# learner-shx/SVG-IR

Measured on AMD Instinct MI355X. Metric: Gaussian-surfels/sec fwd+bwd @800x800 (1 view), higher is better.
Workload: dtype f32; 1 GPU; cfg2: rgss path, P=200000 surfels, 800x800, SH degree 3, S=5, VS=0, fwd+bwd, one view per step per GPU (BASELINE.json configs[1] = cfg2 at N=1; configs[3] = cfg4, view r on rank r, at N>1); num_rendered=673008, parallelism=view-parallel x1, per_rank_cpus=not pinned

## Files before the change

### svg-ir_amd/csrc/render_fwd.hip

```cpp
#include <algorithm>

#include "common.hpp"
#include "shade_tables.hpp"
#include "stage.hpp"
#include "pairstage.hpp"
#include "dev_trace.hpp"

namespace svgir {

namespace {

#ifndef CULL_THREADS
#define CULL_THREADS 256
#endif
constexpr int CT = CULL_THREADS, CNW = CT / 64;

__global__ void __launch_bounds__(CT) cull_kernel(const RenderArgs a) {
    __shared__ uint32_t wcnt[CNW][4];
    const uint32_t tile_u = xcd_tile_of_work(blockIdx.x, a.gx, a.gy);
    if (tile_u == ORDER_NONE) return;
    const int tile = (int)tile_u;
    const uint32_t r0 = a.ranges[2 * tile], r1 = a.ranges[2 * tile + 1];
    const int len = (int)(r1 - r0);
    const int t = threadIdx.x, lane = t & 63, wave = t >> 6;
    const int tx = tile % a.gx, ty = tile / a.gx;
    if (!a.bg_in_render && t < 256 && (a.zero_a || a.zero_b)) {
        const int px = tx * TILE + (t & 15), py = ty * TILE + (t >> 4);
        if (px < a.W && py < a.H) write_zero_planes(a, (size_t)a.W * py + px, (size_t)a.W * a.H);
    }
    if (len == 0) {
        if (t < 4) { a.sub_total[4 * tile + t] = 0u; a.sub_count[4 * tile + t] = 0u; a.sub_ndump[4 * tile + t] = 0u; }
        const int px = tx * TILE + (t & 15), py = ty * TILE + (t >> 4);
        if (!a.bg_in_render && t < 256 && px < a.W && py < a.H) write_background(a, (size_t)a.W * py + px, (size_t)a.W * a.H);
        return;
    }
    const float X0 = (float)(tx * TILE), Y0 = (float)(ty * TILE);
    const float4* __restrict__ rec4 = reinterpret_cast<const float4*>(a.rec);
    uint2* __restrict__ out = a.sub_list + (size_t)4 * r0;
    const unsigned long long lt_mask = (lane == 0) ? 0ull : (~0ull >> (64 - lane));
    uint32_t run[4] = {0u, 0u, 0u, 0u};
    uint32_t gid_n = t < len ? a.point_list[r0 + t] : 0u;
    uint32_t gid_nn = CT + t < len ? a.point_list[r0 + CT + t] : 0u;
    float4 A_n = rec4[(size_t)gid_n * 6], B_n = rec4[(size_t)gid_n * 6 + 1];
    for (int base = 0; base < len; base += CT) {
        const int i = base + t;
        bool m[4] = {false, false, false, false};
        const uint32_t gid = gid_n;
        const float4 A = A_n, B = B_n;
        gid_n = gid_nn;
        if (base + CT < len) { A_n = rec4[(size_t)gid_n * 6]; B_n = rec4[(size_t)gid_n * 6 + 1]; }
        gid_nn = base + 2 * CT + t < len ? a.point_list[r0 + base + 2 * CT + t] : 0u;
        if (i < len) {
            const SplatCull sc = cull_prepare(A.x, A.y, A.z, A.w, B.x, B.y);
#pragma unroll
            for (int w = 0; w < 4; w++) {
                const float x0 = X0 + (float)((w & 1) * 8), y0 = Y0 + (float)((w >> 1) * 8);
                m[w] = cull_test(sc, x0, y0, x0 + 7.f, y0 + 7.f);
            }
        }
        unsigned long long mask[4];
#pragma unroll
        for (int w = 0; w < 4; w++) {
            mask[w] = __ballot(m[w]);
            if (lane == 0) wcnt[wave][w] = (uint32_t)__popcll(mask[w]);
        }
        __syncthreads();
        const uint2 e = make_uint2(gid, (uint32_t)i);
#pragma unroll
        for (int w = 0; w < 4; w++) {
            uint32_t before = 0, all = 0;
#pragma unroll
            for (int v = 0; v < CNW; v++) { const uint32_t c = wcnt[v][w]; all += c; before += v < wave ? c : 0u; }
            if (m[w]) out[(size_t)w * len + run[w] + before + (uint32_t)__popcll(mask[w] & lt_mask)] = e;
            run[w] += all;
        }
        __syncthreads();
    }
    if (t < 4) {
        const uint32_t mine = t == 0 ? run[0] : t == 1 ? run[1] : t == 2 ? run[2] : run[3];
        a.sub_total[4 * tile + t] = mine;
        if (mine == 0u) { a.sub_count[4 * tile + t] = 0u; a.sub_ndump[4 * tile + t] = 0u; }
        if (a.queue_order) dispatch_publish_tile(a, tile, blockIdx.x & 7u, run, t);
    }
}

__global__ void __launch_bounds__(64) dispatch_publish_kernel(const RenderArgs a) {
    uint32_t n_ne;
    (void)dispatch_item(a, 0u, (int)threadIdx.x, &n_ne);
}

template <int S, int VC, bool SVGSS, int WPE>
__global__ void __launch_bounds__(64) __attribute__((amdgpu_waves_per_eu(WPE < 2 ? WPE : 2, WPE)))
render_fwd_kernel(const RenderArgs a) {
    using PG = PairGeom<S, VC>;
    constexpr int CH = PG::CH, PF = PG::PF;
    constexpr int KB = StageGeom<S, VC>::KB, NP = KB / 2;
    static_assert(KB == 4 && CH % KB == 0, "a group = the 4 K-rows of one MFMA");
    extern __shared__ __attribute__((aligned(16))) char smem[];
    float* sD = reinterpret_cast<float*>(smem);
    uint2* sQ = reinterpret_cast<uint2*>(smem + PG::off_q);
    float* sW = reinterpret_cast<float*>(smem + PG::off_w);
    float* sP = reinterpret_cast<float*>(smem + PG::off_p);
    constexpr int PS = PG::PS;

    uint32_t n_ne;
    const uint32_t sid = dispatch_item(a, blockIdx.x, (int)threadIdx.x, &n_ne);
    if (sid == ORDER_NONE) {
        if (a.queue_order) dispatch_idle(a, blockIdx.x - n_ne, gridDim.x - n_ne, (int)threadIdx.x);
        return;
    }
    const int tile = (int)(sid >> 2), sub = (int)(sid & 3u);
    const int tx = tile % a.gx, ty = tile / a.gx;
    const int lane = threadIdx.x;
    const int bx = tx * TILE + (sub & 1) * 8, by = ty * TILE + (sub >> 1) * 8;
    const int px = bx + (lane & 7), py = by + (lane >> 3);
    const bool inside = px < a.W && py < a.H;
    const float pxf = (float)px, pyf = (float)py;
    const f32x2 pxx = {pxf, pxf}, pyy = {pyf, pyf};
    const uint32_t r0 = a.ranges[2 * tile], r1 = a.ranges[2 * tile + 1];
    const int len = (int)(r1 - r0);
    if (len == 0) {
        if (a.bg_in_render && !a.dump_only && inside) {
            write_background(a, (size_t)a.W * py + px, (size_t)a.W * a.H);
// ... 47 lines not shown
#pragma unroll
            for (int mt = 0; mt < 4; mt++) {
                float* d = sP + nq * PS + 16 * mt + 4 * kq;
                d[0] = vacc[mt].x; d[1] = vacc[mt].y; d[2] = vacc[mt].z; d[3] = vacc[mt].w;
            }
            wave_lds_sync();
#pragma unroll
            for (int c = 0; c < VC; c++) vfv[c] = sP[c * PS + lane];
        }
        wave_lds_sync();
    };
    auto chan = [&](int c) -> float { return chv[c]; };
    auto vchan = [&](int c) -> float { return vfv[c]; };
    uint32_t last_walk = 0;

    constexpr int NST = 8 + S + VC;
    const uint32_t dump_base = a.sub_slot_base[sid];
    uint32_t ndump = 0;
    auto dump_state = [&](uint32_t j, bool last) {
        const bool slot = dump_base + j < a.slot_cap;
        if (!slot && !last) return;
        gather_acc();
        if (!slot) return;
        float* d = a.seg_state + ((size_t)(dump_base + j) * NST) * 64 + lane;
        d[0] = T; d[64] = chan(0); d[128] = chan(1); d[192] = chan(2);
        d[256] = surface ? chan(3) : 0.f; d[320] = surface ? chan(4) : 0.f; d[384] = surface ? chan(5) : 0.f; d[448] = D;
#pragma unroll
        for (int ch = 0; ch < S; ch++) d[(8 + ch) * 64] = chan(6 + ch);
#pragma unroll
        for (int ch = 0; ch < VC; ch++) d[(8 + S + ch) * 64] = vchan(ch);
    };

    uint32_t head = 0;
    if (total > 0) {
        for (int i = lane; i < (CH / 2) * PF / 4; i += 64) reinterpret_cast<float4*>(sD)[i] = make_float4(0.f, 0.f, 0.f, 0.f);
        auto load_entries = [&](int b) -> uint2 {
            const int i = b * CH + lane;
            return (lane < CH && i < total) ? list[i] : make_uint2(0u, 0u);
        };
        const int nb = (total + CH - 1) / CH;
        if (lane < CH) sQ[lane] = load_entries(0);
        uint2 e_next = load_entries(1);
        wave_lds_sync();
        PairMap<S, VC> pmap;
        pmap.init(lane);
        PairRegs<S, VC> sr;
        pair_stage_load<S, VC, CH>(sr, pmap, min(CH, total), [&](int s) { return sQ[s].x; }, lane, a.rec, a.features, a.vfeatures);
        bool wave_done = __all(done);
        int nflush = 0;
        auto flush_weights = [&](int bprev) {
            if (lane < nflush) {
                const float* wp = sW + (bprev & 1) * (4 * CH) + lane;
                const float wsum = (wp[0] + wp[CH]) + (wp[2 * CH] + wp[3 * CH]);
                if (wsum != 0.f && !a.dump_only) atomic_add_f32(&a.out_weights[sQ[(bprev & 1) * CH + lane].x], wsum);
            }
        };
        int b = 0;
        for (; b < nb && !wave_done; b++) {
            const int m = min(CH, total - b * CH);
            const uint2* q_cur = sQ + (b & 1) * CH;
            float* w_cur = sW + (b & 1) * (4 * CH);
            wave_lds_sync();
            pair_stage_store<S, VC, CH>(sr, pmap, sD, m, lane);
            flush_weights(b - 1);
            wave_lds_sync();
            if (lane < CH) sQ[((b + 1) & 1) * CH + lane] = e_next;
            e_next = load_entries(b + 2);
            wave_lds_sync();
            if (b + 1 < nb) {
                const uint2* q_nxt = sQ + ((b + 1) & 1) * CH;
                pair_stage_load<S, VC, CH>(sr, pmap, min(CH, total - (b + 1) * CH), [&](int s) { return q_nxt[s].x; }, lane, a.rec,
                                       a.features, a.vfeatures);
            }
            DEV_TRACE_MARK(1);
            int nproc = m;
            for (int c0 = 0; c0 < m; c0 += KB) {
                f32x2 dx[NP], dy[NP];
                f32x4 Gd[NP], Ge[NP];
                float pw[KB], al[KB];
#pragma unroll
                for (int p = 0; p < NP; p++) {
                    const f32x4* P = reinterpret_cast<const f32x4*>(sD + ((c0 >> 1) + p) * PF);
                    const f32x4 G0 = P[0], G1 = P[1], G2 = P[2];
                    Gd[p] = P[3]; Ge[p] = P[4];
                    dx[p] = G0.xy - pxx; dy[p] = G0.zw - pyy;
                    const f32x2 pw2 = pair_power2(G1.xy, G2.xy, G1.zw, dx[p], dy[p]);
                    f32x2 a2;
                    {
#pragma clang fp contract(off)
                        a2 = G2.zw * exp_nonpos2(pw2);
                    }
                    pw[2 * p] = pw2.x; pw[2 * p + 1] = pw2.y;
                    al[2 * p] = fminf(0.99f, a2.x); al[2 * p + 1] = fminf(0.99f, a2.y);
                }
                bool pre[KB];
#pragma unroll
                for (int k = 0; k < KB; k++) pre[k] = pw[k] <= 0.0f && al[k] >= (1.0f / 255.0f);
                float w[KB];
#pragma unroll
                for (int k = 0; k < KB; k++) {
                    const bool live = pre[k] && !done;
                    const float test_T = T * (1.f - al[k]);
                    const bool stop = test_T < 0.0001f;
                    const bool pass = live && !stop;
                    done = done || (live && stop);
                    w[k] = pass ? al[k] * T : 0.f;
// ... 49 lines not shown
                    }
                    wave_lds_sync();
                    {
                        const float bch = sD[((c0 >> 1) + (kq >> 1)) * PF + PG::CH_OFF + (kq & 1) * PG::CHP + nq];
    #pragma unroll
                        for (int mt = 0; mt < 4; mt++)
                            acc[mt] = __builtin_amdgcn_mfma_f32_16x16x4f32(sP[kq * PS + 16 * mt + nq], bch, acc[mt], 0, 0, 0);
                    }
                    if (VC > 0) {
    #pragma unroll
                        for (int k = 0; k < KB; k++) {
                            const float bv = sD[((c0 + k) >> 1) * PF + PG::V_OFF + (k & 1) * PG::VB + kq * PG::VCP + nq];
    #pragma unroll
                            for (int mt = 0; mt < 4; mt++)
                                vacc[mt] = __builtin_amdgcn_mfma_f32_16x16x4f32(sP[(4 + k * 4 + kq) * PS + 16 * mt + nq], bv, vacc[mt], 0, 0, 0);
                        }
                    }
                    wave_lds_sync();
                }
                {
                    const bool o1 = (lane & 1) != 0, o2 = (lane & 2) != 0;
                    const float t01 = (o1 ? w[1] : w[0]) + dpp_f32<0xB1>(o1 ? w[0] : w[1]);
                    const float t23 = (o1 ? w[3] : w[2]) + dpp_f32<0xB1>(o1 ? w[2] : w[3]);
                    float u = (o2 ? t23 : t01) + dpp_f32<0x4E>(o2 ? t01 : t23);
                    u += dpp_f32<0x114>(u);
                    u += dpp_f32<0x118>(u);
                    if ((lane & 12) == 12) w_cur[(lane >> 4) * CH + c0 + (lane & 3)] = u;
                }
                if (__all(done)) { wave_done = true; nproc = min(m, c0 + KB); break; }
            }
            nflush = nproc;
            head += (uint32_t)m;
            DEV_TRACE_MARK(2);
            if (!wave_done && (head & (uint32_t)(SEG - 1)) == 0u) dump_state(ndump++, false);
        }
        wave_lds_sync();
        flush_weights(b - 1);
    }
    if (lane == 0 && !a.dump_only) {
        a.sub_count[sid] = head; a.sub_ndump[sid] = ndump;
        const uint32_t nseg = head != 0 ? min((head + (uint32_t)SEG - 1u) / (uint32_t)SEG, ndump + 1u) : 0u;
        if (nseg != 0) {
            uint32_t* cnt = a.seg_block + (tile >> 8) * SEG_BLOCK_STRIDE;
            const int lc = seg_class(head - (nseg - 1u) * (uint32_t)SEG);
            if (nseg > 1u || lc == 0) atomicAdd(cnt, nseg - (lc == 0 ? 0u : 1u));
            if (lc != 0) atomicAdd(cnt + lc, 1u);
        }
    }
    if (head != 0 && ndump != 0) dump_state(ndump, true);
    else gather_acc();

    if (inside && !a.dump_only) {
        const size_t N_ = (size_t)a.W * a.H;
        const size_t pid = (size_t)a.W * py + px;
        if (a.bg_in_render) write_zero_planes(a, pid, N_);
        T = fminf((float)(1 - 0.000001), T);
        a.final_T[pid] = T;
        a.n_contrib[pid] = last_walk ? (int32_t)(list[last_walk - 1u].y + 1u) : 0;
        a.out_color[pid] = chan(0) + T * a.bg[0];
        a.out_color[N_ + pid] = chan(1) + T * a.bg[1];
        a.out_color[2 * N_ + pid] = chan(2) + T * a.bg[2];
#pragma unroll
        for (int ch = 0; ch < S; ch++) a.out_feature[ch * N_ + pid] = chan(6 + ch);
#pragma unroll
        for (int ch = 0; ch < VC; ch++) a.out_vfeature[ch * N_ + pid] = vchan(ch);
        a.out_normal[pid] = surface ? chan(3) : 0.f;
        a.out_normal[N_ + pid] = surface ? chan(4) : 0.f;
        a.out_normal[2 * N_ + pid] = surface ? chan(5) : 0.f;
        a.out_depth[pid] = normalize_depth ? D / (1.f - T) : D + T * 10.f;
        a.out_opacity[pid] = 1.f - T;
        a.final_D[pid] = D;
    }
    DEV_TRACE_MARK(3);
    DEV_TRACE_END(0, (unsigned)total, head, blockIdx.x);
}

__global__ void __launch_bounds__(64) contrib_prepass_kernel(const RenderArgs a) {
    __shared__ __attribute__((aligned(16))) float sQ[2][32][12];
    __shared__ uint32_t sG[2][64];
    uint32_t n_ne;
    const uint32_t sid = dispatch_item(a, blockIdx.x, (int)threadIdx.x, &n_ne);
    if (sid == ORDER_NONE) return;
    const int tile = (int)(sid >> 2), sub = (int)(sid & 3u);
    const uint32_t r0 = a.ranges[2 * tile], r1 = a.ranges[2 * tile + 1];
    const int len = (int)(r1 - r0);
    if (len == 0) return;
    const int total = (int)a.sub_total[sid];
    if (total == 0) return;
    const int lane = threadIdx.x;
    const int tx = tile % a.gx, ty = tile / a.gx;
    const int px = tx * TILE + (sub & 1) * 8 + (lane & 7), py = ty * TILE + (sub >> 1) * 8 + (lane >> 3);
    const float pxf = (float)px, pyf = (float)py;
    const f32x2 pxx = {pxf, pxf}, pyy = {pyf, pyf};
    const uint2* __restrict__ list = a.sub_list + (size_t)4 * r0 + (size_t)sub * len;
// ... 219 lines not shown
```

### svg-ir_amd/csrc/api.hip

```cpp
#include <algorithm>
#include <cstdarg>
#include <cstdio>
#include <atomic>
#include <cstdlib>
#include <ctime>
#include <memory>
#include <mutex>
#include <string>
#include <vector>

#include "common.hpp"
#include "geom_bwd.hpp"
#include "workload_history.hpp"
#include "depth_sort_plan.hpp"

using namespace svgir;

namespace {

thread_local std::string g_err;
std::atomic<bool> g_prof{false};
WorkloadHistory g_history;
unsigned long long* pinned_words(size_t n) {
    void* ptr = nullptr;
// ... 308 lines not shown
                        sp.training ? 52 : 64, sp.training, p->S, p->VS);
        if (!sp.viewmatrix) return fail(SVGIR_ERR_INVALID, "fused shading needs sp.viewmatrix (packed view-space normals)");
    }
    return 0;
}

CapKey workload_key(const svgir_params* p) {
    int dev_id = 0;
    (void)hipGetDevice(&dev_id);
    return CapKey{dev_id, p->W, p->H, p->P, p->S, p->variant == SVGIR_SVGSS ? p->VS : 0, p->variant, p->workload_scope};
}

bool bin_capacity(size_t bytes, const char* image_blob, int W, int H, int nstate, Wait how, const hipStream_t* stream, ViewCounts* vc) {
    const bool compact = bin_bytes_compact(bytes);
    if (compact || how != Wait::kCaps)
        *vc = resolve_view(image_blob, image_layout(const_cast<char*>(image_blob), W, H).counters, how, stream, compact);
    if (compact) return vc->known && vc->cap_slots >= 0;
    vc->cap_R = binning_capacity_from_bytes(bytes, view_grid(W, H).T, nstate);
    vc->cap_slots = -1;
    return true;
}

template <class A> void camera_args(A& a, const svgir_params* p) {
    a.P = p->P; a.D = p->D; a.M = p->M; a.means3D = p->means3D; a.shs = p->colors_precomp ? nullptr : p->shs;
    a.scales = p->scales; a.rotations = p->rotations; a.view = p->viewmatrix; a.proj = p->projmatrix; a.campos = p->cam_pos;
    a.scale_modifier = p->scale_modifier; a.tanx = p->tan_fovx; a.tany = p->tan_fovy; a.cfg = cfg_ref(p);
    a.focal_x = p->W / (2.0f * p->tan_fovx); a.focal_y = p->H / (2.0f * p->tan_fovy);
}

RenderArgs render_args(const svgir_params* p, const ViewGrid& v, const GeomLayout& G, const ImageLayout& I, const BinLayout& B, int fin) {
    const bool svgss = p->variant == SVGIR_SVGSS;
    RenderArgs ra{};
    ra.W = v.W; ra.H = v.H; ra.gx = v.gx; ra.gy = v.gy; ra.S = p->S; ra.VS = svgss ? p->VS : 0;
    ra.ranges = I.ranges; ra.point_list = B.val[fin]; ra.rec = G.rec; ra.features = p->features; ra.vfeatures = p->vfeatures;
    ra.bg = p->background; ra.cfg = cfg_ref(p);
    ra.sub_list = B.sub_list; ra.sub_total = I.sub_total; ra.sub_order = I.sub_order; ra.sub_count = I.sub_count; ra.sub_ndump = I.sub_ndump;
    ra.sub_pair_base = I.sub_pair_base; ra.sub_slot_base = I.sub_slot_base; ra.disp_ctr = I.disp_ctr; ra.disp_item = I.disp_item;
    ra.seg_list = B.seg_list; ra.seg_desc = B.seg_desc; ra.seg_count = I.counters; ra.seg_block = I.seg_block; ra.seg_state = B.seg_state;
    ra.slot_cap = (uint32_t)std::min<size_t>(B.slot_cap, 0xffffffffu);
    ra.order_n = (int)order_entries(v.gx, v.gy);
    ra.bg_in_render = render_specialised(p->S, ra.VS, svgss) ? 1 : 0;
    ra.final_T = I.final_T; ra.final_D = I.final_D; ra.n_contrib = I.n_contrib;
    return ra;
}
}

extern "C" {

int svgir_abi_version(void) { return SVGIR_ABI_VERSION; }
size_t svgir_geom_bytes(int32_t P) { return geom_layout(nullptr, P).bytes; }
size_t svgir_image_bytes(int32_t W, int32_t H) { return image_layout(nullptr, W, H).bytes; }
size_t svgir_binning_bytes(int32_t R, int32_t W, int32_t H, int32_t S, int32_t VS) {
    return bin_layout(nullptr, binning_capacity(R), view_grid(W, H).T, seg_nstate(S, VS)).bytes;
}
size_t svgir_image_ncontrib_offset(int32_t W, int32_t H) { return image_layout(nullptr, W, H).ncontrib_off; }
size_t svgir_image_ranges_offset(int32_t W, int32_t H) {
    const ImageLayout I = image_layout((char*)256, W, H);
    return (size_t)((char*)I.ranges - (char*)256);
}
size_t svgir_binning_point_list_offset(size_t binning_bytes, const char* image_blob, int32_t W, int32_t H, int32_t S, int32_t VS) {
    const int T = view_grid(W, H).T, nstate = seg_nstate(S, VS);
    ViewCounts vc;
    if (!bin_capacity(binning_bytes, image_blob, W, H, nstate, Wait::kCaps, nullptr, &vc)) return (size_t)-1;
    const BinLayout B = bin_layout((char*)256, vc.cap_R, T, nstate);
    return (size_t)((char*)B.val[tile_sort_plan(T).passes & 1] - (char*)256);
}
// ... 595 lines not shown
```

### svg-ir_amd/csrc/common.hpp

```cpp
#pragma once
#include <hip/hip_runtime.h>
#include <stddef.h>
#include <stdint.h>
#include <stdlib.h>

#include <algorithm>

#include "../../include/svgir_raster.h"
#include "wave.hpp"

namespace svgir {

constexpr int TILE = 16;
constexpr int BLOCK = 256;
constexpr int REC = 24;

enum RecField {
    R_X = 0, R_Y = 1, R_CX = 2, R_CY = 3,
    R_CZ = 4, R_OP = 5, R_DEPTH = 6, R_DA = 7,
    R_J0 = 8, R_J1 = 9, R_J2 = 10, R_J3 = 11,
    R_DB = 12, R_R = 13, R_G = 14, R_B = 15,
    R_NX = 16, R_NY = 17, R_NZ = 18, R_IU = 19,
    R_IV = 20, R_IBASE = 21, R_RECT = 22, R_PAD2 = 23
};
// ... 47 lines not shown
    g.key[0] = (uint32_t*)take(p * 4);
    g.key[1] = (uint32_t*)take(p * 4);
    g.idx[0] = (uint32_t*)take(p * 4);
    g.idx[1] = (uint32_t*)take(p * 4);
    g.offsets = (uint32_t*)take(p * 4);
    g.radix_tbl = (uint32_t*)take(radix_table_words(P) * 4);
    g.radix_wtbl = (uint32_t*)take((size_t)256 * sort_blocks(P) * 4);
    g.counters = (uint32_t*)take(16);
    g.key_top = (uint32_t*)take((p + 63) / 64 * 4);
    g.needed = (uint8_t*)take(p);
    g.shade_list = (uint32_t*)take(p * 4);
    g.shade_work = (uint32_t*)take(((size_t)scan_blocks(P) + 2) * 4);
    g.bytes = off;
    return g;
}

constexpr uint32_t ORDER_NONE = 0xffffffffu;
#if defined(__HIPCC__)
__host__ __device__
#endif
inline uint32_t xcd_of_tile(int tx, int ty) { return (uint32_t)((tx >> 2) + 3 * (ty >> 2)) & 7u; }
inline size_t order_entries(int gx, int gy) {
    size_t cnt[8] = {0, 0, 0, 0, 0, 0, 0, 0};
    for (int by = 0; 4 * by < gy; by++)
        for (int bx = 0; 4 * bx < gx; bx++) cnt[xcd_of_tile(4 * bx, 4 * by)] += (size_t)std::min(4, gx - 4 * bx) * (size_t)std::min(4, gy - 4 * by);
    size_t m = 0;
    for (size_t c : cnt) m = std::max(m, c);
    return std::max((size_t)8 * 4 * m, (size_t)4 * gx * gy);
}

#if defined(__HIPCC__)
__host__ __device__
#endif
inline uint32_t xcd_tile_of_work(uint32_t q, int gx, int gy) {
    const int c = (int)(q & 7u), nbx = (gx + 3) >> 2, nby = (gy + 3) >> 2;
    const int wl = gx - 4 * (nbx - 1);
    uint32_t rem = q >> 3;
    for (int by = 0; by < nby; by++) {
        const int bh = gy - 4 * by < 4 ? gy - 4 * by : 4;
        const int r = (c - 3 * by) & 7;
        const int nblk = nbx > r ? (nbx - r + 7) / 8 : 0;
        const bool has_last = nblk > 0 && ((nbx - 1 - r) & 7) == 0;
        const uint32_t cnt = (uint32_t)(bh * (4 * nblk - (has_last ? 4 - wl : 0)));
        if (rem >= cnt) { rem -= cnt; continue; }
        const int k = (int)(rem / (uint32_t)(bh * 4));
        const int bx = r + 8 * k;
        const uint32_t within = rem - (uint32_t)(k * bh * 4);
        const int bw = bx == nbx - 1 ? wl : 4;
        return (uint32_t)((4 * by + (int)(within / (uint32_t)bw)) * gx + 4 * bx + (int)(within % (uint32_t)bw));
    }
    return ORDER_NONE;
}

constexpr int SEG_CLASSES = 5, SEG_BLOCK_STRIDE = 8;

struct ImageLayout {
    float* final_T;
    float* final_D;
    int32_t* n_contrib;
    uint32_t* ranges;
    uint32_t* seg_block;
    uint32_t* sub_total;
    uint32_t* sub_order;
    uint32_t* sub_count;
    uint32_t* sub_ndump;
    uint32_t* sub_pair_base;
    uint32_t* sub_slot_base;
    uint32_t* counters;
    uint32_t* disp_ctr;
    uint32_t* disp_item;
    size_t ncontrib_off;
    size_t bytes;
};
constexpr int DISP_NCLS = 64, DISP_SHARDS = 8, DISP_STEP = 16;
constexpr int DISP_CTR_WORDS = DISP_NCLS * DISP_SHARDS + 2;
inline ImageLayout image_layout(char* base, int W, int H) {
    ImageLayout im;
    size_t off = 0;
    auto take = [&](size_t bytes) { char* p = base ? base + off : nullptr; off += align_up(bytes); return p; };
    const size_t N = (size_t)W * H;
    const size_t T = (size_t)((W + TILE - 1) / TILE) * ((H + TILE - 1) / TILE);
    im.final_T = (float*)take(N * 4);
    im.final_D = (float*)take(N * 4);
    im.ncontrib_off = off;
// ... 133 lines not shown
    return i < c.len && c.ptr[i] > 0.f;
}
#endif

struct ShadeTables {
    const float* env = nullptr; float4* env_tab = nullptr; int ntexel = 0, softplus = 0;
    int Ns = 0; float4* lat_tab = nullptr;
    float* zero = nullptr; int nzero = 0;
#if defined(__HIPCC__)
    __host__ __device__
#endif
    int entries() const { return env ? (ntexel > (lat_tab ? Ns : 0) ? ntexel : (lat_tab ? Ns : 0)) : 0; }
};

struct PreArgs {
    int P, D, M, W, H, gx, gy;
    const float *means3D, *shs, *colors_precomp, *opacities, *scales, *rotations, *cov3D_precomp;
    const float *view, *proj, *campos, *patchbbox;
    float scale_modifier, tanx, tany, focal_x, focal_y;
    CfgRef cfg;
    float* rec; float* cov3D; uint32_t* clamped; uint32_t* tiles; uint32_t* key; uint32_t* idx; int32_t* radii;
    float* out_weights;
    uint8_t* needed;
    uint32_t* span;
    ShadeTables tabs; int pblocks;
    uint32_t* zero_words; int n_zero_words;
    int spec_top; uint32_t* key_top;
    uint32_t* prefilter_violation;
    const float* features; int embed_S;
};

struct RenderArgs {
    int W, H, gx, gy, S, VS;
    const uint32_t* ranges; const uint32_t* point_list;
    const float* rec; const float* features; const float* vfeatures;
    const float* bg;
    CfgRef cfg;
    uint2* sub_list; uint32_t* sub_total; uint32_t* sub_order; uint32_t* sub_count;
    uint32_t* sub_ndump; uint32_t* seg_list; SegDesc* seg_desc; uint32_t* seg_count; uint32_t* seg_block; float* seg_state;
    uint32_t* sub_pair_base; uint32_t* sub_slot_base; uint32_t slot_cap;
    int bg_in_render;
    int order_n;
    int hi_fill;
    int dump_only;
    float *final_T, *final_D; int32_t* n_contrib;
    float *out_color, *out_normal, *out_depth, *out_opacity, *out_feature, *out_vfeature, *out_weights;
    float *zero_a, *zero_b;
    uint8_t* needed;
    int queue_order; uint32_t* disp_ctr; uint32_t* disp_item;
    int publish; uint32_t pub_tag, pub_cap_R, pub_magic; long long pub_cap_slots; unsigned long long* pub_host;
};

struct RenderBwdArgs {
    int W, H, gx, gy, S, VS;
    const uint32_t* ranges; const uint32_t* point_list;
    const float* rec; const float* features; const float* vfeatures;
    const float* bg;
    CfgRef cfg; int backward_geometry;
    const uint2* sub_list; const uint32_t* sub_count;
    const uint32_t* sub_ndump; const uint32_t* seg_list; const SegDesc* seg_desc; const uint32_t* seg_count; const float* seg_state; int seg_cap;
    const float *final_T, *final_D; const int32_t* n_contrib;
    const float *g_color, *g_normal, *g_depth, *g_opacity, *g_feature, *g_vfeature;
    float *dL_dmean2D, *dL_dconic, *dL_dopacity, *dL_dcolor, *dL_dfeature, *dL_dvfeature, *dL_dnormal, *dL_ddepth;
    float* grad_rows; uint32_t* row_of; uint32_t rows_cap;
    uint4* clear; size_t clear_n16;
};
// ... 205 lines not shown
```

### svg-ir_amd/csrc/stage.hpp

```cpp
#pragma once
#include "common.hpp"

namespace svgir {

template <int S, int VC>
struct StageGeom {
    static constexpr int S4 = (S + 3) / 4 * 4;
    static constexpr int NFD = REC + S4 + VC * 4;
    static constexpr int NF4 = (NFD / 4) | 1;
    static constexpr int NF = NF4 * 4;
    static constexpr int C4 = 6 + VC;
    static constexpr int CH = NF <= 48 ? 64 : 32;
    static constexpr int QN = 2 * CH;
#ifndef FWD_KB_V
#define FWD_KB_V 4
#endif
#ifndef FWD_KB_P
#define FWD_KB_P 4
#endif
    static constexpr int KB = VC > 0 ? FWD_KB_V : FWD_KB_P;
#ifndef FWD_WPE_V
#define FWD_WPE_V 2
#endif
#ifndef FWD_WPE_P
// ... 6 lines not shown
    static_assert(SEG % CH == 0, "segment boundaries must fall on staging-batch boundaries");
    static_assert(CH % KB == 0, "a staging batch is a whole number of blend batches");
};

#if defined(__HIPCC__)
__device__ __forceinline__ float pair_power(float a, float b, float c, float dx, float dy) {
    float s, m;
    {
#pragma clang fp contract(off)
        s = a * dx * dx + c * dy * dy;
        m = b * dx * dy;
    }
    return __builtin_fmaf(-0.5f, s, -m);
}

__device__ __forceinline__ float exp_nonpos(float x) {
    const float L2E_HI = 1.44269502162933349609375f;
    const float L2E_LO = 1.92596299112661746e-8f;
    const float t = x * L2E_HI;
    float r = __builtin_fmaf(x, L2E_HI, -t);
    r = __builtin_fmaf(x, L2E_LO, r);
    const float e = __builtin_amdgcn_exp2f(t);
    return __builtin_fmaf(e, r * 0.693147182464599609375f, e);
}

struct SplatCull {
    float mx, my, a, b, c, tau2, ia, ic;
    bool degenerate;
};
__device__ __forceinline__ SplatCull cull_prepare(float mx, float my, float a, float b, float c, float op) {
    SplatCull s;
    s.mx = mx; s.my = my; s.a = a; s.b = b; s.c = c;
    s.tau2 = 2.f * 0.693147182f * __builtin_amdgcn_logf(255.f * op);
    s.degenerate = !(a > 0.f) || !(c > 0.f) || !(a * c - b * b > 0.f);
    s.ia = __builtin_amdgcn_rcpf(a); s.ic = __builtin_amdgcn_rcpf(c);
    return s;
}
__device__ __forceinline__ bool cull_test(const SplatCull& s, float X0, float Y0, float X1, float Y1) {
    const float u0 = s.mx - X1, u1 = s.mx - X0, v0 = s.my - Y1, v1 = s.my - Y0;
    const float a = s.a, b = s.b, c = s.c;
    const bool in = (u0 <= 0.f) && (u1 >= 0.f) && (v0 <= 0.f) && (v1 >= 0.f);
    float v, u, q, qmin;
    v = fminf(v1, fmaxf(v0, -b * u0 * s.ic)); qmin = a * u0 * u0 + 2.f * b * u0 * v + c * v * v;
    v = fminf(v1, fmaxf(v0, -b * u1 * s.ic)); q = a * u1 * u1 + 2.f * b * u1 * v + c * v * v; qmin = fminf(qmin, q);
    u = fminf(u1, fmaxf(u0, -b * v0 * s.ia)); q = a * u * u + 2.f * b * u * v0 + c * v0 * v0; qmin = fminf(qmin, q);
    u = fminf(u1, fmaxf(u0, -b * v1 * s.ia)); q = a * u * u + 2.f * b * u * v1 + c * v1 * v1; qmin = fminf(qmin, q);
    qmin = in ? 0.f : qmin;
    const float um = fmaxf(fabsf(u0), fabsf(u1)), vm = fmaxf(fabsf(v0), fabsf(v1));
    const float slack = 0.02f + 4e-5f * (a * um * um + 2.f * fabsf(b) * um * vm + c * vm * vm);
    return s.degenerate ? (s.tau2 == s.tau2) : (qmin <= s.tau2 + slack);
}

typedef float f32x4 __attribute__((ext_vector_type(4)));

template <int S, int VC, int CHN>
struct StageRegs {
    using SG = StageGeom<S, VC>;
    static constexpr int KV = (CHN * SG::C4 + 63) / 64;
    static constexpr int KF = (CHN * S + 63) / 64;
    f32x4 v[KV];
    float fv[KF > 0 ? KF : 1];
};

template <int S, int VC, int CHN, typename GidOf>
__device__ __forceinline__ void stage_load(StageRegs<S, VC, CHN>& r, int m, GidOf gid_of, int lane,
                                           const float* __restrict__ rec, const float* __restrict__ feat,
                                           const float* __restrict__ vfeat) {
    using SG = StageGeom<S, VC>;
    using SR = StageRegs<S, VC, CHN>;
    const f32x4* rec4 = reinterpret_cast<const f32x4*>(rec);
    const f32x4* vf4 = reinterpret_cast<const f32x4*>(vfeat);
    const int total = m * SG::C4;
#pragma unroll
    for (int u = 0; u < SR::KV; u++) {
        const int k = min(u * 64 + lane, total - 1);
        const int s = k / SG::C4, part = k - s * SG::C4;
        const size_t id = (size_t)gid_of(s);
        const f32x4* src = part < 6 ? rec4 + id * 6 + part : vf4 + id * VC + (part - 6);
        r.v[u] = *src;
    }
    if (S > 0) {
        const int totf = m * S;
#pragma unroll
// ... 55 lines not shown
```

Measured before the change: 671.0 million surfels/s.

## Defer weight atomics via buffer atomics and overlap dump and epilogue loads

Splits the per-batch weight flush into an LDS read and a later buffer atomic_fadd, issued after the next batch's stage load so the atomic overlaps compute. Inactive lanes are masked by pointing the atomic at an out-of-range offset instead of branching. The segment state dump is deferred into the next iteration, and the n_contrib list entry and bg values are loaded early so their latency is hidden. This adds an explicit waitcnt and more live registers, and it depends on buffer out-of-bounds semantics to drop masked atomics.

```diff
diff --git a/svg-ir_amd/csrc/render_fwd.hip b/svg-ir_amd/csrc/render_fwd.hip
--- a/svg-ir_amd/csrc/render_fwd.hip
+++ b/svg-ir_amd/csrc/render_fwd.hip
@@ -89,6 +89,14 @@
     (void)dispatch_item(a, 0u, (int)threadIdx.x, &n_ne);
 }
 
+constexpr uint32_t WEIGHTS_OFF_NONE = 0xfffffffcu;
+__device__ __forceinline__ __amdgpu_buffer_rsrc_t weights_resource(float* out_weights) {
+    return __builtin_amdgcn_make_buffer_rsrc(out_weights, 0, (int)WEIGHTS_OFF_NONE, 0x00020000);
+}
+__device__ __forceinline__ void weights_atomic(__amdgpu_buffer_rsrc_t res, uint32_t byte_off, float v) {
+    __builtin_amdgcn_raw_ptr_buffer_atomic_fadd_f32(v, res, (int)byte_off, 0, 0);
+}
+
 template <int S, int VC, bool SVGSS, int WPE>
 __global__ void __launch_bounds__(64) __attribute__((amdgpu_waves_per_eu(WPE < 2 ? WPE : 2, WPE)))
 render_fwd_kernel(const RenderArgs a) {
@@ -202,6 +210,12 @@
     };
 
     uint32_t head = 0;
+    bool dump_pending = false;
+    uint32_t nc_last = 0u;
+    float fl_w = 0.f;
+    uint32_t fl_g = 0u;
+    const __amdgpu_buffer_rsrc_t wres = weights_resource(a.out_weights);
+    auto flush_issue = [&]() { weights_atomic(wres, (fl_w != 0.f && !a.dump_only) ? fl_g * 4u : WEIGHTS_OFF_NONE, fl_w); };
     if (total > 0) {
         for (int i = lane; i < (CH / 2) * PF / 4; i += 64) reinterpret_cast<float4*>(sD)[i] = make_float4(0.f, 0.f, 0.f, 0.f);
         auto load_entries = [&](int b) -> uint2 {
@@ -218,21 +232,25 @@
         pair_stage_load<S, VC, CH>(sr, pmap, min(CH, total), [&](int s) { return sQ[s].x; }, lane, a.rec, a.features, a.vfeatures);
         bool wave_done = __all(done);
         int nflush = 0;
-        auto flush_weights = [&](int bprev) {
+        auto flush_read = [&](int bprev) {
+            fl_w = 0.f;
             if (lane < nflush) {
                 const float* wp = sW + (bprev & 1) * (4 * CH) + lane;
-                const float wsum = (wp[0] + wp[CH]) + (wp[2 * CH] + wp[3 * CH]);
-                if (wsum != 0.f && !a.dump_only) atomic_add_f32(&a.out_weights[sQ[(bprev & 1) * CH + lane].x], wsum);
+                fl_w = (wp[0] + wp[CH]) + (wp[2 * CH] + wp[3 * CH]);
+                fl_g = sQ[(bprev & 1) * CH + lane].x;
             }
         };
+        flush_issue();
         int b = 0;
         for (; b < nb && !wave_done; b++) {
             const int m = min(CH, total - b * CH);
             const uint2* q_cur = sQ + (b & 1) * CH;
             float* w_cur = sW + (b & 1) * (4 * CH);
             wave_lds_sync();
+            flush_read(b - 1);
+            __builtin_amdgcn_s_waitcnt(0x0F71);
             pair_stage_store<S, VC, CH>(sr, pmap, sD, m, lane);
-            flush_weights(b - 1);
+            if (dump_pending) { dump_state(ndump++, false); dump_pending = false; }
             wave_lds_sync();
             if (lane < CH) sQ[((b + 1) & 1) * CH + lane] = e_next;
             e_next = load_entries(b + 2);
@@ -242,6 +260,7 @@
                 pair_stage_load<S, VC, CH>(sr, pmap, min(CH, total - (b + 1) * CH), [&](int s) { return q_nxt[s].x; }, lane, a.rec,
                                        a.features, a.vfeatures);
             }
+            flush_issue();
             DEV_TRACE_MARK(1);
             int nproc = m;
             for (int c0 = 0; c0 < m; c0 += KB) {
@@ -357,11 +376,16 @@
             nflush = nproc;
             head += (uint32_t)m;
             DEV_TRACE_MARK(2);
-            if (!wave_done && (head & (uint32_t)(SEG - 1)) == 0u) dump_state(ndump++, false);
-        }
+            dump_pending = !wave_done && (head & (uint32_t)(SEG - 1)) == 0u;
+        }
+        if (last_walk) nc_last = list[last_walk - 1u].y;
         wave_lds_sync();
-        flush_weights(b - 1);
-    }
+        flush_read(b - 1);
+    }
+    const float bg0 = a.bg[0], bg1 = a.bg[1], bg2 = a.bg[2];
+    asm volatile("" :: "v"(nc_last), "v"(bg0), "v"(bg1), "v"(bg2));
+    if (dump_pending) dump_state(ndump++, false);
+    flush_issue();
     if (lane == 0 && !a.dump_only) {
         a.sub_count[sid] = head; a.sub_ndump[sid] = ndump;
         const uint32_t nseg = head != 0 ? min((head + (uint32_t)SEG - 1u) / (uint32_t)SEG, ndump + 1u) : 0u;
@@ -381,10 +405,10 @@
         if (a.bg_in_render) write_zero_planes(a, pid, N_);
         T = fminf((float)(1 - 0.000001), T);
         a.final_T[pid] = T;
-        a.n_contrib[pid] = last_walk ? (int32_t)(list[last_walk - 1u].y + 1u) : 0;
-        a.out_color[pid] = chan(0) + T * a.bg[0];
-        a.out_color[N_ + pid] = chan(1) + T * a.bg[1];
-        a.out_color[2 * N_ + pid] = chan(2) + T * a.bg[2];
+        a.n_contrib[pid] = last_walk ? (int32_t)(nc_last + 1u) : 0;
+        a.out_color[pid] = chan(0) + T * bg0;
+        a.out_color[N_ + pid] = chan(1) + T * bg1;
+        a.out_color[2 * N_ + pid] = chan(2) + T * bg2;
 #pragma unroll
         for (int ch = 0; ch < S; ch++) a.out_feature[ch * N_ + pid] = chan(6 + ch);
 #pragma unroll
```

Measured after the change: 675.4 million surfels/s (median of 6 runs). No clear change (+0.7%).

## Streamline cull kernel: magic-divide tile mapping, packed counts, deferred stores, one barrier

Applied to the files above, without the earlier changes.

Replaces the loop-based XCD tile-order decode with a closed-form group computation that uses a magic-number divide passed in through RenderArgs. The cull kernel now packs the four per-wave survivor counts into 16-bit fields, double-buffers the shared counters so each round needs one barrier instead of two, and defers each round's output stores into the next iteration. The cull test is rewritten to share per-corner products across the four 8x8 sub-quads and uses explicit FMAs with contraction disabled. The aim is to cut scalar integer work, barriers and redundant float math in a kernel dominated by per-tile overhead. The risks are small floating-point differences in the cull decision and more live registers.

```diff
diff --git a/svg-ir_amd/csrc/api.hip b/svg-ir_amd/csrc/api.hip
--- a/svg-ir_amd/csrc/api.hip
+++ b/svg-ir_amd/csrc/api.hip
@@ -364,6 +364,7 @@
     const bool svgss = p->variant == SVGIR_SVGSS;
     RenderArgs ra{};
     ra.W = v.W; ra.H = v.H; ra.gx = v.gx; ra.gy = v.gy; ra.S = p->S; ra.VS = svgss ? p->VS : 0;
+    ra.xcd_magic = xcd_group_magic(v.gx, v.gy);
     ra.ranges = I.ranges; ra.point_list = B.val[fin]; ra.rec = G.rec; ra.features = p->features; ra.vfeatures = p->vfeatures;
     ra.bg = p->background; ra.cfg = cfg_ref(p);
     ra.sub_list = B.sub_list; ra.sub_total = I.sub_total; ra.sub_order = I.sub_order; ra.sub_count = I.sub_count; ra.sub_ndump = I.sub_ndump;
diff --git a/svg-ir_amd/csrc/common.hpp b/svg-ir_amd/csrc/common.hpp
--- a/svg-ir_amd/csrc/common.hpp
+++ b/svg-ir_amd/csrc/common.hpp
@@ -103,24 +103,50 @@
 #if defined(__HIPCC__)
 __host__ __device__
 #endif
+inline uint32_t xcd_group_magic(int gx, int gy) {
+    const unsigned long long d = 4ull * (unsigned long long)gx;
+    return (unsigned long long)gx * (unsigned long long)gy * d < (1ull << 32) ? (uint32_t)(((1ull << 32) + d - 1ull) / d) : 0u;
+}
+#if defined(__HIPCC__)
+__host__ __device__
+#endif
+inline uint32_t div_1to4(uint32_t x, uint32_t d) { return d == 3u ? (x * 43691u) >> 17 : x >> (d >> 1); }
+#if defined(__HIPCC__)
+__host__ __device__
+#endif
+inline uint32_t xcd_tile_of_work(uint32_t q, int gx, int gy, uint32_t magic, int* tx, int* ty) {
+    const uint32_t nbx = (uint32_t)(gx + 3) >> 2;
+    const uint32_t wl = (uint32_t)gx - 4u * (nbx - 1u);
+    const uint32_t extra = nbx & 7u, rl = (nbx - 1u) & 7u, w0 = 4u * (nbx >> 3);
+    const uint32_t d = 4u * (uint32_t)gx;
+    uint32_t rem = q >> 3;
+    const uint32_t g = magic ? (uint32_t)(((unsigned long long)rem * magic) >> 32) : rem / d;
+    rem -= g * d;
+    int rows = gy - (int)(32u * g);
+    uint32_t r = q & 7u;
+    uint32_t bh, by = 8u * g;
+    for (const uint32_t end = by + 8u;; by++, rows -= 4, r = (r + 5u) & 7u) {
+        if (by == end || rows <= 0) return ORDER_NONE;
+        bh = rows < 4 ? (uint32_t)rows : 4u;
+        const uint32_t cnt = bh * (w0 + (r < extra ? 4u : 0u) - (r == rl ? 4u - wl : 0u));
+        if (rem < cnt) break;
+        rem -= cnt;
+    }
+    const uint32_t k = div_1to4(rem >> 2, bh);
+    const uint32_t bx = r + 8u * k;
+    const uint32_t within = rem - k * bh * 4u;
+    const uint32_t bw = bx == nbx - 1u ? wl : 4u;
+    const uint32_t row = div_1to4(within, bw);
+    *tx = (int)(4u * bx + (within - row * bw));
+    *ty = (int)(4u * by + row);
+    return (uint32_t)(*ty * gx + *tx);
+}
+#if defined(__HIPCC__)
+__host__ __device__
+#endif
 inline uint32_t xcd_tile_of_work(uint32_t q, int gx, int gy) {
-    const int c = (int)(q & 7u), nbx = (gx + 3) >> 2, nby = (gy + 3) >> 2;
-    const int wl = gx - 4 * (nbx - 1);
-    uint32_t rem = q >> 3;
-    for (int by = 0; by < nby; by++) {
-        const int bh = gy - 4 * by < 4 ? gy - 4 * by : 4;
-        const int r = (c - 3 * by) & 7;
-        const int nblk = nbx > r ? (nbx - r + 7) / 8 : 0;
-        const bool has_last = nblk > 0 && ((nbx - 1 - r) & 7) == 0;
-        const uint32_t cnt = (uint32_t)(bh * (4 * nblk - (has_last ? 4 - wl : 0)));
-        if (rem >= cnt) { rem -= cnt; continue; }
-        const int k = (int)(rem / (uint32_t)(bh * 4));
-        const int bx = r + 8 * k;
-        const uint32_t within = rem - (uint32_t)(k * bh * 4);
-        const int bw = bx == nbx - 1 ? wl : 4;
-        return (uint32_t)((4 * by + (int)(within / (uint32_t)bw)) * gx + 4 * bx + (int)(within % (uint32_t)bw));
-    }
-    return ORDER_NONE;
+    int tx, ty;
+    return xcd_tile_of_work(q, gx, gy, xcd_group_magic(gx, gy), &tx, &ty);
 }
 
 constexpr int SEG_CLASSES = 5, SEG_BLOCK_STRIDE = 8;
@@ -320,6 +346,7 @@
 
 struct RenderArgs {
     int W, H, gx, gy, S, VS;
+    uint32_t xcd_magic;
     const uint32_t* ranges; const uint32_t* point_list;
     const float* rec; const float* features; const float* vfeatures;
     const float* bg;
diff --git a/svg-ir_amd/csrc/render_fwd.hip b/svg-ir_amd/csrc/render_fwd.hip
--- a/svg-ir_amd/csrc/render_fwd.hip
+++ b/svg-ir_amd/csrc/render_fwd.hip
@@ -16,14 +16,16 @@
 constexpr int CT = CULL_THREADS, CNW = CT / 64;
 
 __global__ void __launch_bounds__(CT) cull_kernel(const RenderArgs a) {
-    __shared__ uint32_t wcnt[CNW][4];
-    const uint32_t tile_u = xcd_tile_of_work(blockIdx.x, a.gx, a.gy);
+    __shared__ uint2 wcnt[2][CNW];
+    static_assert(CT < 65536, "the survivors of a round are summed in 16-bit fields");
+    DEV_TRACE_DECL();
+    int tx, ty;
+    const uint32_t tile_u = xcd_tile_of_work(blockIdx.x, a.gx, a.gy, a.xcd_magic, &tx, &ty);
     if (tile_u == ORDER_NONE) return;
     const int tile = (int)tile_u;
     const uint32_t r0 = a.ranges[2 * tile], r1 = a.ranges[2 * tile + 1];
     const int len = (int)(r1 - r0);
-    const int t = threadIdx.x, lane = t & 63, wave = t >> 6;
-    const int tx = tile % a.gx, ty = tile / a.gx;
+    const int t = threadIdx.x, lane = t & 63, wave = __builtin_amdgcn_readfirstlane(t >> 6);
     if (!a.bg_in_render && t < 256 && (a.zero_a || a.zero_b)) {
         const int px = tx * TILE + (t & 15), py = ty * TILE + (t >> 4);
         if (px < a.W && py < a.H) write_zero_planes(a, (size_t)a.W * py + px, (size_t)a.W * a.H);
@@ -37,51 +39,61 @@
     const float X0 = (float)(tx * TILE), Y0 = (float)(ty * TILE);
     const float4* __restrict__ rec4 = reinterpret_cast<const float4*>(a.rec);
     uint2* __restrict__ out = a.sub_list + (size_t)4 * r0;
-    const unsigned long long lt_mask = (lane == 0) ? 0ull : (~0ull >> (64 - lane));
     uint32_t run[4] = {0u, 0u, 0u, 0u};
     uint32_t gid_n = t < len ? a.point_list[r0 + t] : 0u;
     uint32_t gid_nn = CT + t < len ? a.point_list[r0 + CT + t] : 0u;
     float4 A_n = rec4[(size_t)gid_n * 6], B_n = rec4[(size_t)gid_n * 6 + 1];
-    for (int base = 0; base < len; base += CT) {
+    unsigned long long pmask[4] = {0ull, 0ull, 0ull, 0ull};
+    uint32_t ppos[4] = {0u, 0u, 0u, 0u};
+    uint2 pe = make_uint2(0u, 0u);
+    auto store_previous = [&]() {
+#pragma unroll
+        for (int w = 0; w < 4; w++)
+            if (__builtin_amdgcn_inverse_ballot_w64(pmask[w])) (out + (size_t)w * len)[ppos[w]] = pe;
+    };
+    DEV_TRACE_MARK(0);
+    for (int base = 0, buf = 0; base < len; base += CT, buf ^= 1) {
         const int i = base + t;
-        bool m[4] = {false, false, false, false};
         const uint32_t gid = gid_n;
-        const float4 A = A_n, B = B_n;
+        float4 A = A_n, B = B_n;
+        asm volatile("" : "+v"(A.x), "+v"(A.y), "+v"(A.z), "+v"(A.w), "+v"(B.x), "+v"(B.y));
+        store_previous();
         gid_n = gid_nn;
         if (base + CT < len) { A_n = rec4[(size_t)gid_n * 6]; B_n = rec4[(size_t)gid_n * 6 + 1]; }
         gid_nn = base + 2 * CT + t < len ? a.point_list[r0 + base + 2 * CT + t] : 0u;
-        if (i < len) {
-            const SplatCull sc = cull_prepare(A.x, A.y, A.z, A.w, B.x, B.y);
-#pragma unroll
-            for (int w = 0; w < 4; w++) {
-                const float x0 = X0 + (float)((w & 1) * 8), y0 = Y0 + (float)((w >> 1) * 8);
-                m[w] = cull_test(sc, x0, y0, x0 + 7.f, y0 + 7.f);
-            }
-        }
         unsigned long long mask[4];
+        cull_test_tile(cull_prepare(A.x, A.y, A.z, A.w, B.x, B.y), X0, Y0, i < len, mask);
+        if (lane == 0)
+            wcnt[buf][wave] = make_uint2((uint32_t)__popcll(mask[0]) | ((uint32_t)__popcll(mask[1]) << 16),
+                                         (uint32_t)__popcll(mask[2]) | ((uint32_t)__popcll(mask[3]) << 16));
+        __syncthreads();
+        uint2 before = make_uint2(0u, 0u), all = make_uint2(0u, 0u);
+#pragma unroll
+        for (int v = 0; v < CNW; v++) {
+            const uint2 c = wcnt[buf][v];
+            all.x += c.x; all.y += c.y;
+            before.x += v < wave ? c.x : 0u; before.y += v < wave ? c.y : 0u;
+        }
+        pe = make_uint2(gid, (uint32_t)i);
 #pragma unroll
         for (int w = 0; w < 4; w++) {
-            mask[w] = __ballot(m[w]);
-            if (lane == 0) wcnt[wave][w] = (uint32_t)__popcll(mask[w]);
-        }
-        __syncthreads();
-        const uint2 e = make_uint2(gid, (uint32_t)i);
-#pragma unroll
-        for (int w = 0; w < 4; w++) {
-            uint32_t before = 0, all = 0;
-#pragma unroll
-            for (int v = 0; v < CNW; v++) { const uint32_t c = wcnt[v][w]; all += c; before += v < wave ? c : 0u; }
-            if (m[w]) out[(size_t)w * len + run[w] + before + (uint32_t)__popcll(mask[w] & lt_mask)] = e;
-            run[w] += all;
-        }
-        __syncthreads();
-    }
+            const uint32_t bw = w & 1 ? (w & 2 ? before.y : before.x) >> 16 : (w & 2 ? before.y : before.x) & 0xffffu;
+            const uint32_t aw = w & 1 ? (w & 2 ? all.y : all.x) >> 16 : (w & 2 ? all.y : all.x) & 0xffffu;
+            ppos[w] = __builtin_amdgcn_mbcnt_hi((uint32_t)(mask[w] >> 32), __builtin_amdgcn_mbcnt_lo((uint32_t)mask[w], run[w] + bw));
+            pmask[w] = mask[w];
+            run[w] += aw;
+        }
+    }
+    store_previous();
+    DEV_TRACE_MARK(1);
     if (t < 4) {
         const uint32_t mine = t == 0 ? run[0] : t == 1 ? run[1] : t == 2 ? run[2] : run[3];
         a.sub_total[4 * tile + t] = mine;
         if (mine == 0u) { a.sub_count[4 * tile + t] = 0u; a.sub_ndump[4 * tile + t] = 0u; }
         if (a.queue_order) dispatch_publish_tile(a, tile, blockIdx.x & 7u, run, t);
     }
+    DEV_TRACE_MARK(2);
+    DEV_TRACE_END(1, (unsigned)len, (unsigned)((len + CT - 1) / CT), blockIdx.x);
 }
 
 __global__ void __launch_bounds__(64) dispatch_publish_kernel(const RenderArgs a) {
diff --git a/svg-ir_amd/csrc/stage.hpp b/svg-ir_amd/csrc/stage.hpp
--- a/svg-ir_amd/csrc/stage.hpp
+++ b/svg-ir_amd/csrc/stage.hpp
@@ -62,23 +62,62 @@
     SplatCull s;
     s.mx = mx; s.my = my; s.a = a; s.b = b; s.c = c;
     s.tau2 = 2.f * 0.693147182f * __builtin_amdgcn_logf(255.f * op);
-    s.degenerate = !(a > 0.f) || !(c > 0.f) || !(a * c - b * b > 0.f);
+    {
+#pragma clang fp contract(off)
+        s.degenerate = !(a > 0.f) || !(c > 0.f) || !(a * c > b * b);
+    }
     s.ia = __builtin_amdgcn_rcpf(a); s.ic = __builtin_amdgcn_rcpf(c);
     return s;
 }
-__device__ __forceinline__ bool cull_test(const SplatCull& s, float X0, float Y0, float X1, float Y1) {
-    const float u0 = s.mx - X1, u1 = s.mx - X0, v0 = s.my - Y1, v1 = s.my - Y0;
-    const float a = s.a, b = s.b, c = s.c;
-    const bool in = (u0 <= 0.f) && (u1 >= 0.f) && (v0 <= 0.f) && (v1 >= 0.f);
-    float v, u, q, qmin;
-    v = fminf(v1, fmaxf(v0, -b * u0 * s.ic)); qmin = a * u0 * u0 + 2.f * b * u0 * v + c * v * v;
-    v = fminf(v1, fmaxf(v0, -b * u1 * s.ic)); q = a * u1 * u1 + 2.f * b * u1 * v + c * v * v; qmin = fminf(qmin, q);
-    u = fminf(u1, fmaxf(u0, -b * v0 * s.ia)); q = a * u * u + 2.f * b * u * v0 + c * v0 * v0; qmin = fminf(qmin, q);
-    u = fminf(u1, fmaxf(u0, -b * v1 * s.ia)); q = a * u * u + 2.f * b * u * v1 + c * v1 * v1; qmin = fminf(qmin, q);
-    qmin = in ? 0.f : qmin;
-    const float um = fmaxf(fabsf(u0), fabsf(u1)), vm = fmaxf(fabsf(v0), fabsf(v1));
-    const float slack = 0.02f + 4e-5f * (a * um * um + 2.f * fabsf(b) * um * vm + c * vm * vm);
-    return s.degenerate ? (s.tau2 == s.tau2) : (qmin <= s.tau2 + slack);
+__device__ __forceinline__ void cull_test_tile(const SplatCull& s, float X0, float Y0, bool valid, unsigned long long mask[4]) {
+#pragma clang fp contract(off)
+    const float a = s.a, c = s.c, b2 = 2.f * s.b, nb = -s.b, ab2 = 2.f * fabsf(s.b);
+    float u[4], v[4], au[4], bu[4], tv[4], cv[4], tu[4];
+#pragma unroll
+    for (int h = 0; h < 2; h++) {
+        const float x0 = X0 + (float)(8 * h), y0 = Y0 + (float)(8 * h);
+        u[2 * h] = s.mx - (x0 + 7.f); u[2 * h + 1] = s.mx - x0;
+        v[2 * h] = s.my - (y0 + 7.f); v[2 * h + 1] = s.my - y0;
+    }
+#pragma unroll
+    for (int e = 0; e < 4; e++) {
+        au[e] = a * u[e]; bu[e] = b2 * u[e]; tv[e] = nb * u[e] * s.ic;
+        cv[e] = c * v[e]; tu[e] = nb * v[e] * s.ia;
+    }
+    bool inx[2], iny[2];
+    float aum[2], bum[2], um[2], cvm[2], vm[2];
+#pragma unroll
+    for (int h = 0; h < 2; h++) {
+        inx[h] = u[2 * h] <= 0.f && u[2 * h + 1] >= 0.f;
+        iny[h] = v[2 * h] <= 0.f && v[2 * h + 1] >= 0.f;
+        um[h] = fmaxf(fabsf(u[2 * h]), fabsf(u[2 * h + 1])); vm[h] = fmaxf(fabsf(v[2 * h]), fabsf(v[2 * h + 1]));
+        aum[h] = a * um[h]; bum[h] = ab2 * um[h]; cvm[h] = c * vm[h];
+    }
+    const unsigned long long regular = __builtin_amdgcn_ballot_w64(valid && !s.degenerate);
+    const unsigned long long kept = __builtin_amdgcn_ballot_w64(valid && s.degenerate && s.tau2 == s.tau2);
+#pragma unroll
+    for (int w = 0; w < 4; w++) {
+        const int hx = w & 1, hy = w >> 1;
+        const float u0 = u[2 * hx], u1 = u[2 * hx + 1], v0 = v[2 * hy], v1 = v[2 * hy + 1];
+        float qmin = 0.f;
+#pragma unroll
+        for (int k = 0; k < 2; k++) {
+            const int e = 2 * hx + k;
+            const float y = fminf(v1, fmaxf(v0, tv[e]));
+            const float q = __builtin_fmaf(y, c * y, __builtin_fmaf(u[e], au[e], bu[e] * y));
+            qmin = k == 0 ? q : fminf(qmin, q);
+        }
+#pragma unroll
+        for (int k = 0; k < 2; k++) {
+            const int e = 2 * hy + k;
+            const float x = fminf(u1, fmaxf(u0, tu[e]));
+            const float q = __builtin_fmaf(v[e], cv[e], __builtin_fmaf(x, a * x, b2 * x * v[e]));
+            qmin = fminf(qmin, q);
+        }
+        qmin = inx[hx] && iny[hy] ? 0.f : qmin;
+        const float slack = __builtin_fmaf(4e-5f, __builtin_fmaf(vm[hy], cvm[hy], __builtin_fmaf(um[hx], aum[hx], bum[hx] * vm[hy])), 0.02f);
+        mask[w] = (__builtin_amdgcn_ballot_w64(qmin <= s.tau2 + slack) & regular) | kept;
+    }
 }
 
 typedef float f32x4 __attribute__((ext_vector_type(4)));
```

Measured after the change: 668.1 million surfels/s before, 674.3 million surfels/s after (median of 6 runs). About the same (+0.9%).
